# knagrecha/saturn

Measured on NVIDIA H100. Metric: candidate schedules/sec, higher is better.
Workload: dtype f32

## Files before the change

### include/saturn_b200.h

```cpp
#ifndef SATURN_B200_H
#define SATURN_B200_H

#include <stddef.h>
#include <stdint.h>

#ifdef __cplusplus
extern "C" {
#endif

#define SB_ABI_VERSION 1
#define SB_NSLOT 8
#define SB_MAX_STRATEGIES 32
#define SB_MAX_NODES 8

typedef enum sb_status {
  SB_OK = 0,
  SB_ERR_ARG = -1,
  SB_ERR_CUDA = -2,
  SB_ERR_STATE = -3,
  SB_ERR_UNSUPPORTED = -4,
  SB_ERR_NOMEM = -5
} sb_status;

#define SB_FLAG_INTEGER_STARTS 1u
// ... 78 lines not shown
  double* history_wall_s;
  int64_t* history_evaluated;
  float* history_makespan;
} sb_search_control;
typedef struct sb_search_result {
  float makespan;
  uint64_t key;
  int64_t evaluated;
  int rounds;
  int stop_reason;
  double wall_s;
} sb_search_result;
int sb_search_seed_lpt(sb_handle* h);
int sb_search_run(sb_handle* h, const sb_search_params* p, const sb_search_control* c, const uint8_t* warm_opt,
                  const void* warm_prio, uint8_t* opt_out , void* prio_out ,
                  sb_search_result* result);
int sb_search_run_multi(sb_handle** handles, int n, const sb_search_params* p, const sb_search_control* c,
                        const uint8_t* warm_opt, const void* warm_prio, uint8_t* opt_out ,
                        void* prio_out , sb_search_result* result);
int sb_search_wave(sb_handle* h, unsigned flags, int64_t* chains);
int sb_search_is_fused(sb_handle* h);
int sb_search_validate(sb_handle* h, int64_t* bad_rows);
int sb_search_verify_count(sb_handle* h, uint64_t* mismatches);
int sb_search_stats(sb_handle* h, int64_t* evaluated, int64_t* rounds_done);

#ifdef __cplusplus
}
#endif
#endif
```

### saturn_b200/_lib.py

```python
import ctypes as C
import os

_HERE = os.path.dirname(os.path.abspath(__file__))
SO_PATH = os.environ.get("SATURN_B200_LIB") or os.path.join(_HERE, "libsaturn_b200.so")

FLAG_INTEGER_STARTS = 1
FLAG_REDUCED = 2
FLAG_OPT_BY_POSITION = 4
FLAG_POST_KEY = 8
FLAG_FOLD_PREV = 16
FLAG_ALT_WARPSCAN = 32
FLAG_SUM_COMPLETION = 64
FLAG_WEIGHTED = 128
FLAG_DUE = 256
FLAG_RELEASE = 512
IPC_HANDLE_BYTES = 64
HOOK_FORCE_GENERIC = 0x80000000
HOOK_NO_STREAM = 0x40000000
HOOK_NO_FUSED = 0x20000000
HOOK_NO_INCREMENTAL = 0x10000000
HOOK_VERIFY_INCREMENTAL = 0x08000000
HOOK_ROUND1_MOVES = 0x04000000
HOOK_PLAIN_ADDR = 0x02000000
HOOK_WINDOW_BIAS = 0x01000000
HOOK_TABLE_GLOBAL = 0x00800000
HOOK_TABLE_PAIR = 0x00400000
HOOK_REORDER = 0x00200000
HOOK_NO_REORDER = 0x00100000

SYMBOLS = [
    "sb_abi_version", "sb_last_error", "sb_create", "sb_destroy", "sb_sync", "sb_set_table",
    "sb_set_sentinel", "sb_set_weights", "sb_set_due", "sb_set_release", "sb_get_reduced", "sb_eval", "sb_last_eval_path", "sb_validate", "sb_eval_host", "sb_eval_full",
    "sb_decode", "sb_xchg_create", "sb_xchg_connect", "sb_xchg_connect_local", "sb_xchg_post", "sb_xchg_reduce", "sb_xchg_check",
    "sb_search_init", "sb_search_round", "sb_search_best_key_ptr", "sb_search_best",
    "sb_search_inject", "sb_search_resample", "sb_search_seed_lpt", "sb_search_run", "sb_search_run_multi", "sb_search_wave", "sb_search_is_fused", "sb_search_stats", "sb_search_validate", "sb_search_verify_count",
]


class SearchParams(C.Structure):
    _fields_ = [("seed", C.c_uint64), ("chains", C.c_int64), ("chain_base", C.c_uint64),
                ("flags", C.c_uint), ("t_start", C.c_float), ("t_end", C.c_float),
                ("total_rounds", C.c_int), ("resample_every", C.c_int)]


class SearchControl(C.Structure):
    _fields_ = [("rounds", C.c_int), ("resample_every", C.c_int), ("sync_every", C.c_int), ("patience", C.c_int),
                ("heuristic_seeds", C.c_int), ("target_makespan", C.c_float), ("time_budget_s", C.c_double),
                ("history_cap", C.c_int), ("history_len", C.POINTER(C.c_int)),
                ("history_wall_s", C.POINTER(C.c_double)), ("history_evaluated", C.POINTER(C.c_int64)),
                ("history_makespan", C.POINTER(C.c_float))]


class SearchResultC(C.Structure):
    _fields_ = [("makespan", C.c_float), ("key", C.c_uint64), ("evaluated", C.c_int64), ("rounds", C.c_int),
                ("stop_reason", C.c_int), ("wall_s", C.c_double)]


class SaturnB200Error(RuntimeError):
# ... 33 lines not shown
        "sb_decode": [vp, vp, vp, u32, vp, vp, vp, vp, vp, vp],
        "sb_xchg_create": [vp, ci, ci, vp],
        "sb_xchg_connect": [vp, vp],
        "sb_xchg_connect_local": [C.POINTER(vp), ci],
        "sb_xchg_post": [vp, vp],
        "sb_xchg_reduce": [vp, vp, vp],
        "sb_xchg_check": [vp],
        "sb_search_init": [vp, C.POINTER(SearchParams), vp, vp],
        "sb_search_round": [vp, ci],
        "sb_search_best_key_ptr": [vp, C.POINTER(vp)],
        "sb_search_best": [vp, vp, vp, C.POINTER(C.c_float), C.POINTER(C.c_uint64)],
        "sb_search_inject": [vp, vp, vp, i64, ci],
        "sb_search_resample": [vp],
        "sb_search_seed_lpt": [vp],
        "sb_search_run": [vp, C.POINTER(SearchParams), C.POINTER(SearchControl), vp, vp, vp, vp,
                          C.POINTER(SearchResultC)],
        "sb_search_run_multi": [C.POINTER(vp), ci, C.POINTER(SearchParams), C.POINTER(SearchControl), vp, vp, vp, vp,
                                C.POINTER(SearchResultC)],
        "sb_search_wave": [vp, C.c_uint, C.POINTER(i64)],
        "sb_search_is_fused": [vp],
        "sb_search_stats": [vp, C.POINTER(i64), C.POINTER(i64)],
        "sb_search_validate": [vp, C.POINTER(i64)],
        "sb_search_verify_count": [vp, C.POINTER(C.c_uint64)],
    }
    for name, args in sigs.items():
        fn = getattr(lib, name)
        fn.argtypes = args
        fn.restype = ci
    _lib = lib
    return lib


def check(rc):
    if rc != 0:
        msg = load().sb_last_error()
        raise SaturnB200Error("saturn_b200 error %d: %s" % (rc, msg.decode() if msg else "?"))
```

### saturn_b200/csrc/sb_api.cu

```cuda
#include <math.h>
#include <stdarg.h>
#include <stdio.h>
#include <string.h>

#include <algorithm>
#include <chrono>
#include <new>
#include <string>
#include <thread>
#include <utility>
#include <vector>

#include "sb_search.h"

using namespace sb;

static thread_local char g_err[512] = "";

static int fail(int code, const char* fmt, ...) {
  va_list ap;
  va_start(ap, fmt);
  vsnprintf(g_err, sizeof(g_err), fmt, ap);
  va_end(ap);
  return code;
// ... 26 lines not shown
  bool win = false, inc = false, verify = false;
  SearchDev alloc;
  const float* w = nullptr;
  const float* due = nullptr;
  const float* rel = nullptr;
};

struct sb_handle {
  Device dev;
  cudaStream_t stream = nullptr;
  bool own_stream = false;
  int J = 0, S = 0;
  int tab_J = 0, tab_S = 0;
  int nodes = 1;
  float sentinel = kSentinel;
  float* tab = nullptr;
  float* tmin = nullptr;
  uint8_t* args = nullptr;
  uint8_t* vopt[2] = {nullptr, nullptr};
  int* nvalid[2] = {nullptr, nullptr};
  std::vector<float> h_tmin;
  std::vector<uint8_t> h_args;
  unsigned long long* d_scratch = nullptr;
  uint8_t* by_pos = nullptr;
  size_t by_pos_bytes = 0;
  cudaStream_t hs[2] = {nullptr, nullptr};
  uint8_t* st_o[2] = {nullptr, nullptr};
  uint8_t* st_p[2] = {nullptr, nullptr};
  float* st_mk[2] = {nullptr, nullptr};
  long long st_cap = 0;
  size_t st_row_o = 0, st_row_p = 0;
  uint8_t* dec_buf = nullptr;
  size_t dec_cap = 0;
  float* stage_T = nullptr;
  size_t stage_T_bytes = 0;
  float* d_w = nullptr;
  size_t d_w_cap = 0;
  std::vector<float> h_w;
  double w_sum = 0.0;
  bool has_w = false;
  float* d_d = nullptr;
  float* d_one = nullptr;
  size_t d_d_cap = 0;
  std::vector<float> h_d;
  bool has_d = false;
  float* d_r = nullptr;
// ... 87 lines not shown
  h->dev.ordinal = device;
  h->dev.sm_count = prop.multiProcessorCount;
  h->dev.smem_optin = prop.sharedMemPerBlockOptin;
  h->stream = static_cast<cudaStream_t>(stream);
  e = cudaMalloc(&h->d_scratch, 4 * sizeof(unsigned long long));
  if (e != cudaSuccess) { sb_destroy(h); return fail(SB_ERR_CUDA, "cudaMalloc: %s", cudaGetErrorString(e)); }
  for (int i = 0; i < 2; ++i) {
    e = cudaStreamCreateWithFlags(&h->hs[i], cudaStreamNonBlocking);
    if (e != cudaSuccess) { sb_destroy(h); return fail(SB_ERR_CUDA, "cudaStreamCreate: %s", cudaGetErrorString(e)); }
  }
  *out = h;
  return SB_OK;
}

int sb_destroy(sb_handle* h) {
  if (!h) return SB_OK;
  cudaSetDevice(h->dev.ordinal);
  cudaStreamSynchronize(h->stream);
  free_search(h);
  free_table(h);
  free_staging(h);
  free_xchg(h);
  cudaFree(h->d_scratch);
  cudaFree(h->by_pos);
  cudaFree(h->dec_buf);
  cudaFree(h->stage_T);
  cudaFree(h->d_w);
  cudaFree(h->d_d);
  cudaFree(h->d_one);
  cudaFree(h->d_r);
  cudaFree(h->d_rc);
  for (int i = 0; i < 2; ++i)
    if (h->hs[i]) cudaStreamDestroy(h->hs[i]);
  if (h->own_stream && h->stream) cudaStreamDestroy(h->stream);
  delete h;
  return SB_OK;
}

int sb_sync(sb_handle* h) {
  int rc = use_device(h);
  if (rc) return rc;
  CK(cudaStreamSynchronize(h->stream));
  return SB_OK;
}

int sb_set_table(sb_handle* h, const float* T, const uint8_t* gcount, int J, int S, int G, int nodes) {
// ... 287 lines not shown
      cp.opt = h->by_pos;
      int path = 5;
      CK(eval_pos_launch(h->dev, cp, h->stream, &path));
      h->last_path = 9;
      return SB_OK;
    }
  }
  if (flags & SB_FLAG_ALT_WARPSCAN) {
    if (flags & (SB_FLAG_SUM_COMPLETION | SB_FLAG_WEIGHTED | SB_FLAG_DUE | SB_FLAG_RELEASE))
      return fail(SB_ERR_UNSUPPORTED, "SB_FLAG_ALT_WARPSCAN scores the makespan without release dates only: it "
                  "cannot be combined with SB_FLAG_SUM_COMPLETION, SB_FLAG_WEIGHTED, SB_FLAG_DUE or SB_FLAG_RELEASE");
    if (flags & (SB_FLAG_POST_KEY | SB_FLAG_FOLD_PREV))
      return fail(SB_ERR_UNSUPPORTED, "SB_FLAG_ALT_WARPSCAN cannot be combined with the fused key exchange");
    cudaError_t e = eval_alt_launch(h->dev, c, h->stream);
    if (e == cudaErrorNotSupported) {
      cudaGetLastError();
      return fail(SB_ERR_UNSUPPORTED, "SB_FLAG_ALT_WARPSCAN needs one node and a table that fits in shared memory");
    }
    CK(e);
    h->last_path = 6;
    return SB_OK;
  }
  c.force_generic = (flags & HOOK_FORCE_GENERIC) ? 1 : 0;
  const bool post = (flags & SB_FLAG_POST_KEY) != 0;
  if (post) {
    if (!h->xchg_ready) return fail(SB_ERR_STATE, "SB_FLAG_POST_KEY needs sb_xchg_connect first");
    if (!best_key) return fail(SB_ERR_ARG, "SB_FLAG_POST_KEY needs best_key");
    c.xp.x = h->xd;
    c.xp.seq = ++h->xseq;
    c.xp.counter = h->d_xcounter;
    c.xp.fold_prev = (flags & SB_FLAG_FOLD_PREV) ? 1 : 0;
    c.xp.error = h->d_xerr;
  }
  CK(eval_launch(h->dev, c, h->stream, &h->last_path));
  if (post && (h->last_path == 0 || B == 0)) {
    if (c.xp.fold_prev && h->xseq > 1)
      CK(xchg_reduce_launch(h->xd, h->xseq - 1, h->d_scratch + 1, reinterpret_cast<unsigned long long*>(best_key),
                            h->d_xerr, h->stream));
    CK(xchg_post_launch(h->xd, reinterpret_cast<unsigned long long*>(best_key), h->xseq, h->stream));
  }
  return SB_OK;
}

int sb_last_eval_path(sb_handle* h) { return h ? h->last_path : -1; }

int sb_validate(sb_handle* h, const uint8_t* opt, const void* prio, int64_t B, int64_t row_stride, unsigned flags,
// ... 887 lines not shown
  CK(validate_launch(h->dev, c, h->d_scratch, h->stream, s.d.pos != 0));
  unsigned long long bad = 0;
  CK(cudaMemcpyAsync(&bad, h->d_scratch, sizeof(bad), cudaMemcpyDeviceToHost, h->stream));
  CK(cudaStreamSynchronize(h->stream));
  *bad_rows = static_cast<int64_t>(bad);
  return SB_OK;
}

int sb_search_verify_count(sb_handle* h, uint64_t* mismatches) {
  int rc = use_device(h);
  if (rc) return rc;
  if (!mismatches) return fail(SB_ERR_ARG, "mismatches is null");
  SearchState& s = h->search;
  if (!s.ready) return fail(SB_ERR_STATE, "sb_search_init has not been called");
  *mismatches = 0;
  if (!s.verify_bad) return SB_OK;
  unsigned long long v = 0;
  CK(cudaMemcpyAsync(&v, s.verify_bad, sizeof(v), cudaMemcpyDeviceToHost, h->stream));
  CK(cudaStreamSynchronize(h->stream));
  *mismatches = v;
  return SB_OK;
}

int sb_search_is_fused(sb_handle* h) { return (h && h->search.ready && h->search.fused_ok) ? 1 : 0; }

int sb_search_stats(sb_handle* h, int64_t* evaluated, int64_t* rounds_done) {
  if (!h) return fail(SB_ERR_ARG, "null handle");
  if (evaluated) *evaluated = h->search.evaluated;
  if (rounds_done) *rounds_done = h->search.rounds_done;
  return SB_OK;
}

}
```

### saturn_b200/csrc/sb_common.cuh

```cuda
#pragma once
#include <cuda_runtime.h>
#include <stdint.h>

#include "../../include/saturn_b200.h"

#if defined(__CUDA_ARCH__) && (__CUDA_ARCH__ != 900)
#error "saturn_b200 kernels target sm_90a (H100) only"
#endif

namespace sb {

constexpr int kSlots = SB_NSLOT;
constexpr int kWarp = 32;
constexpr int kMaxNodes = SB_MAX_NODES;
constexpr float kSentinel = 1.0e6f;

__device__ __forceinline__ float inf_f() { return __int_as_float(0x7f800000); }

__device__ __forceinline__ uint32_t smem_u32(const void* p) {
  return static_cast<uint32_t>(__cvta_generic_to_shared(p));
}
__device__ __forceinline__ uint32_t cluster_ctarank() {
  uint32_t r;
  asm volatile("mov.u32 %0, %%cluster_ctarank;" : "=r"(r));
// ... 26 lines not shown
  uint32_t ok;
  asm volatile(
      "{\n\t.reg .pred p;\n\t"
      "mbarrier.try_wait.parity.shared::cta.b64 p, [%1], %2;\n\t"
      "selp.u32 %0, 1, 0, p;\n\t}"
      : "=r"(ok)
      : "r"(smem_u32(bar)), "r"(parity)
      : "memory");
  return ok != 0;
}
__device__ __forceinline__ void mbar_wait(uint64_t* bar, uint32_t parity) {
  uint32_t spins = 0;
  while (!mbar_try_wait(bar, parity)) {
    if (++spins > (1u << 26)) __trap();
  }
}
__device__ __forceinline__ void tma_bulk_g2s(void* dst_smem, const void* src_gmem, uint32_t bytes,
                                             uint64_t* bar) {
  asm volatile(
      "cp.async.bulk.shared::cluster.global.mbarrier::complete_tx::bytes [%0], [%1], %2, [%3];" ::"r"(
          smem_u32(dst_smem)),
      "l"(src_gmem), "r"(bytes), "r"(smem_u32(bar))
      : "memory");
}

__device__ __forceinline__ void pmov_fma(float& dst, float src, int bit, int one) {
  int d = __float_as_int(dst);
  asm("{\n\t.reg .pred p;\n\tsetp.ne.s32 p, %2, 0;\n\t@p mad.lo.s32 %0, %1, %3, 0;\n\t}"
      : "+r"(d)
      : "r"(__float_as_int(src)), "r"(bit), "r"(one));
  dst = __int_as_float(d);
}
__device__ __forceinline__ void pinf_fma(float& dst, int bit) {
  asm("{\n\t.reg .pred p;\n\tsetp.ne.s32 p, %1, 0;\n\t@p add.f32 %0, %0, 0f7F800000;\n\t}" : "+f"(dst) : "r"(bit));
}
__device__ __forceinline__ float psel(float a, float b, int bit) {
  float r;
  asm("{\n\t.reg .pred p;\n\tsetp.ne.s32 p, %3, 0;\n\tselp.f32 %0, %1, %2, p;\n\t}" : "=f"(r) : "f"(a), "f"(b), "r"(bit));
  return r;
}

__device__ __forceinline__ float fmax3_mk(float mk, float b, float c) {
  return __int_as_float(__vimax3_s32(__float_as_int(mk), __float_as_int(b), __float_as_int(c)));
}

template <bool kIntegerStarts, bool kTrackMk = kIntegerStarts, bool kSum = false, bool kWeighted = false,
// ... 58 lines not shown
```

### saturn_b200/csrc/sb_eval.cu

```cuda
#include "sb_lane.cuh"

namespace sb {

struct TileArgs {
  const float* tab;
  int J, SG;
  const uint8_t* opt;
  const uint8_t* prio;
  long long B;
  long long stride_o, stride_p;
  int row_o, row_p;
  int copy_o, copy_p;
  int use_bulk;
  int nodes;
  float* out;
  unsigned long long* best_key;
  uint32_t id_base;
  long long ntiles;
  int one;
  SearchFuse sf;
  XchgPost xp;
  const float* w;
  const float* d;
  const float* r;
};

template <int PB, bool INT, bool STREAM, bool MULTI, bool SEARCH = false, bool TABG = false, int ADDR = 0,
          bool SUM = false, bool W = false, bool D = false, bool R = false>
__global__ void __launch_bounds__(STREAM ? 512 : 384, 1) k_eval_tiles(const TileArgs a) {
  static_assert(!(SEARCH && (STREAM || TABG)), "the fused search round runs on shared-memory tiles only");
  static_assert(ADDR == 0 || (!TABG && !MULTI && !SEARCH), "ADDR = 1 needs the table and the opt rows in shared memory");
  static_assert(SUM || !W, "weights scale the sum of completion times only");
  static_assert(W || !D, "due dates run on the weighted form");
  extern __shared__ __align__(128) uint8_t smem[];
  const int nw = blockDim.x >> 5;
  const int warp = threadIdx.x >> 5, lane = threadIdx.x & 31;
  const uint32_t tab_bytes = TABG ? 0u : static_cast<uint32_t>(a.J) * a.SG * 4u;
  const uint32_t w_bytes = (W && !TABG) ? ((static_cast<uint32_t>(a.J) * 4u + 15u) & ~15u) : 0u;
  const uint32_t d_bytes = D ? w_bytes : 0u;
  const uint32_t r_bytes = (R && !TABG) ? ((static_cast<uint32_t>(a.J) * 4u + 15u) & ~15u) : 0u;
  float* tab_s = reinterpret_cast<float*>(smem);
  [[maybe_unused]] float* w_s = reinterpret_cast<float*>(smem + tab_bytes);
  [[maybe_unused]] float* d_s = reinterpret_cast<float*>(smem + tab_bytes + w_bytes);
  [[maybe_unused]] float* r_s = reinterpret_cast<float*>(smem + tab_bytes + w_bytes + d_bytes);
  uint64_t* bars = reinterpret_cast<uint64_t*>(smem + ((tab_bytes + w_bytes + d_bytes + r_bytes + 15u) & ~15u));
  uint8_t* tiles = reinterpret_cast<uint8_t*>(bars) + (((1 + nw) * 8 + 15) & ~15);
  const uint32_t node_bytes = MULTI ? static_cast<uint32_t>(a.nodes) * 1024u : 0u;
// ... 88 lines not shown
    unsigned long long k = ~0ull;
    bool ok = true;
    if (lane < a.xp.x.world) {
      const unsigned long long* slot = a.xp.x.peer[lane] + (want & 1ull) * 2;
      unsigned long long seen;
      unsigned spins = 0;
      for (;;) {
        asm volatile("ld.acquire.sys.global.u64 %0, [%1];" : "=l"(seen) : "l"(slot + 1) : "memory");
        if (seen >= want || !block || ++spins >= (1u << 22)) break;
        __nanosleep(64);
      }
      ok = seen >= want;
      if (ok) asm volatile("ld.relaxed.sys.global.u64 %0, [%1];" : "=l"(k) : "l"(slot) : "memory");
    }
    ok = __all_sync(0xffffffffu, ok);
    if (!ok) {
      if (block && lane == 0) *a.xp.error = 1;
      return;
    }
    fold_keys(k);
  };
  if (fold_pending) look_issue();

  uint32_t phase = 0;
  bool tab_ready = TABG;
  for (long long tile = static_cast<long long>(blockIdx.x) * nw + warp; tile < a.ntiles;
       tile += static_cast<long long>(gridDim.x) * nw) {
    const long long b0 = tile * 32;
    if (!SEARCH && fold_pending) {
      look_consume();
      if (fold_pending) look_issue();
    }
    const long long cand = (SEARCH && a.sf.deal) ? lane * a.ntiles + tile : b0 + lane;
    const bool active = cand < a.B;
    const int nb = SEARCH ? __popc(__ballot_sync(0xffffffffu, active)) : static_cast<int>(min(32ll, a.B - b0));
    const uint8_t* pg = a.prio + cand * a.stride_p;
    __syncwarp();
    PrioChunk q;
    if (a.use_bulk) {
      fence_proxy_async();
      if (lane == 0)
        mbar_arrive_expect_tx(bar_w, static_cast<uint32_t>(nb) * (a.copy_o + (STREAM ? 0 : a.copy_p)));
      __syncwarp();
      if (active) {
        tma_bulk_g2s(tile_o + lane * a.row_o, a.opt + cand * a.stride_o, a.copy_o, bar_w);
        if (!STREAM) tma_bulk_g2s(tile_p + lane * a.row_p, pg, a.copy_p, bar_w);
      }
      if (STREAM && active) q = ld_prio32<true>(pg);
      mbar_wait(bar_w, phase);
      phase ^= 1;
    } else {
      for (int r = 0; r < nb; ++r) {
        const uint8_t* so = a.opt + (b0 + r) * a.stride_o;
        const uint8_t* sp = a.prio + (b0 + r) * a.stride_p;
        for (int x = lane; x < a.J; x += 32) tile_o[r * a.row_o + x] = so[x];
        for (int x = lane; x < a.J * PB; x += 32) tile_p[r * a.row_p + x] = sp[x];
      }
      __syncwarp();
    }
    if (!tab_ready) {
      mbar_wait(bar_tab, 0);
      tab_ready = true;
    }
    auto evaluate = [&](const uint8_t* prio_row_s) -> float {
      st.reset(a.nodes);
      const int J = a.J;
      if constexpr (STREAM && ADDR == 1) {
        constexpr int STEPS = 32;
        constexpr int kBatch = 8;
        const int nch = (J + STEPS - 1) / STEPS, nfull = J / STEPS;
        uint32_t ob[kBatch];
        float rb[kBatch];
        [[maybe_unused]] float wb[kBatch];
// ... 1 lines not shown
        [[maybe_unused]] float xb[kBatch];
        auto resolve = [&](const uint32_t* w) {
          int js[kBatch];
#pragma unroll
          for (int i = 0; i < kBatch; ++i) js[i] = prio_at<1>(w, i);
#pragma unroll
          for (int i = 0; i < kBatch; ++i) ob[i] = st.gather_opt(js[i]);
#pragma unroll
          for (int i = 0; i < kBatch; ++i) rb[i] = st.gather_rt(js[i], ob[i]);
          if constexpr (W) {
#pragma unroll
            for (int i = 0; i < kBatch; ++i) wb[i] = st.gather_w(js[i]);
          }
          if constexpr (D) {
#pragma unroll
            for (int i = 0; i < kBatch; ++i) db[i] = st.gather_d(js[i]);
          }
          if constexpr (R) {
#pragma unroll
            for (int i = 0; i < kBatch; ++i) xb[i] = st.gather_r(js[i]);
          }
        };
        if (nfull > 0) resolve(q.w);
        for (int c = 0; c < nfull; ++c) {
          PrioChunk nxt = q;
          if (c + 1 < nch) nxt = ld_prio32<true>(pg + (c + 1) * 32);
          const bool ahead = c + 1 < nfull;
          uint32_t head[kBatch / 4];
#pragma unroll
          for (int i = 0; i < kBatch / 4; ++i) head[i] = ahead ? nxt.w[i] : q.w[i];
#pragma unroll
          for (int b = 0; b < STEPS / kBatch; ++b) {
            uint32_t oc[kBatch];
            float rc[kBatch];
            [[maybe_unused]] float wc[kBatch];
            [[maybe_unused]] float dc[kBatch];
            [[maybe_unused]] float xc[kBatch];
#pragma unroll
            for (int i = 0; i < kBatch; ++i) { oc[i] = ob[i]; rc[i] = rb[i]; }
            if constexpr (W) {
#pragma unroll
              for (int i = 0; i < kBatch; ++i) wc[i] = wb[i];
            }
            if constexpr (D) {
#pragma unroll
              for (int i = 0; i < kBatch; ++i) dc[i] = db[i];
            }
            if constexpr (R) {
#pragma unroll
              for (int i = 0; i < kBatch; ++i) xc[i] = xb[i];
            }
            resolve(b + 1 < STEPS / kBatch ? q.w + (b + 1) * (kBatch / 4) : head);
#pragma unroll
            for (int i = 0; i < kBatch; ++i) {
              const float x = R ? xc[i] : 0.f;
              if constexpr (D) st.step_resolved(static_cast<int>(oc[i]), rc[i], i & 1, wc[i], dc[i], x);
              else if constexpr (W) st.step_resolved(static_cast<int>(oc[i]), rc[i], i & 1, wc[i], 0.f, x);
              else st.step_resolved(static_cast<int>(oc[i]), rc[i], i & 1, 0.f, 0.f, x);
            }
          }
          q = nxt;
        }
        if (nfull < nch) {
          const int rem = J - nfull * STEPS;
#pragma unroll
          for (int t = 0; t < STEPS; ++t)
            if (t < rem) st.step(prio_at<1>(q.w, t), t & 1);
        }
      } else if (STREAM) {
        constexpr int STEPS = 32 / PB;
        const int nch = (J + STEPS - 1) / STEPS;
        for (int c = 0; c < nch; ++c) {
          PrioChunk nxt = q;
          if (c + 1 < nch) nxt = ld_prio32<true>(pg + (c + 1) * 32);
          if ((c + 1) * STEPS <= J) {
#pragma unroll
            for (int t = 0; t < STEPS; ++t) st.step(prio_at<PB>(q.w, t), t & 1);
          } else {
            const int rem = J - c * STEPS;
#pragma unroll
            for (int t = 0; t < STEPS; ++t)
              if (t < rem) st.step(prio_at<PB>(q.w, t), t & 1);
          }
          q = nxt;
        }
      } else {
        const uint4* prow = reinterpret_cast<const uint4*>(prio_row_s);
        constexpr int STEPS = 16 / PB;
        const int nch = (J + STEPS - 1) / STEPS;
        for (int c = 0; c < nch; ++c) {
          const uint4 p = prow[c];
          const uint32_t w[4] = {p.x, p.y, p.z, p.w};
          if ((c + 1) * STEPS <= J) {
#pragma unroll
            for (int t = 0; t < STEPS; ++t) st.step(prio_at<PB>(w, t), t & 1);
          } else {
            const int rem = J - c * STEPS;
#pragma unroll
            for (int t = 0; t < STEPS; ++t)
              if (t < rem) st.step(prio_at<PB>(w, t), t & 1);
          }
        }
      }
      return st.result();
    };
    [[maybe_unused]] auto eval_from = [&](const uint8_t* prio_row_s, int w0, uint32_t par, bool save,
                                          float* snap_t) -> float {
// ... 20 lines not shown
          for (int i = 0; i < 8; ++i) __stcg(sp + i * 32, st.f[i]);
          __stcg(sp + 8 * 32, st.running());
        }
        const uint4 p = prow[c];
        const uint32_t wd[4] = {p.x, p.y, p.z, p.w};
        if ((c + 1) * STEPS <= J) {
#pragma unroll
          for (int t = 0; t < STEPS; ++t) st.step(prio_at<PB>(wd, t), t & 1);
        } else {
          const int rem = J - c * STEPS;
#pragma unroll 1
          for (int t = 0; t < rem; ++t) st.step(PB == 1 ? prio_row_s[c * STEPS + t] : reinterpret_cast<const uint16_t*>(prio_row_s)[c * STEPS + t], -1);
        }
      }
      return st.result();
    };
    if (!SEARCH) {
      float mk = 0.f;
      if (active) {
        mk = evaluate(tile_p + lane * a.row_p);
        a.out[b0 + lane] = mk;
      }
      if (a.best_key != nullptr) fold_best(a.best_key, active, mk, a.id_base + static_cast<uint32_t>(b0 + lane), lane);
    } else {
      const long long c = cand;
      const int rl = active ? lane : 0;
      uint8_t* orow_s = tile_o + rl * a.row_o;
      uint8_t* prow_s = tile_p + rl * a.row_p;
      st.orow = orow_s;
      const uint64_t gid = a.sf.chain_base + static_cast<uint64_t>(c);
      float cm = active ? a.sf.cur_mk[c] : 0.f;
      bool moving = active;
      const bool inc = !MULTI && a.sf.snap != nullptr;
      const bool win = !MULTI && a.sf.win != 0;
      const int nwin = (a.J + kSnapPos - 1) / kSnapPos;
      float* snap_t = inc ? a.sf.snap + static_cast<size_t>(tile) * (static_cast<size_t>(nwin - 1) * 2 * 9 * 32) : nullptr;
      uint32_t par = 0;
      const uint32_t inc_bits = launch_incumbent_bits(a.sf);
#pragma unroll 1
      for (int r = inc ? -1 : 0; r < a.sf.nrounds; ++r) {
        const int round = a.sf.round + r;
        const bool fill = r < 0;
        if (!fill && a.sf.resample_every > 0 && round > 1 && (round - 1) % a.sf.resample_every == 0) {
          const uint64_t rr = rng_u64(a.sf.seed ^ 0x7e57a11ull, gid, static_cast<uint64_t>(round));
          const int rival = static_cast<int>(rr >> 59);
          const float rcm = __shfl_sync(0xffffffffu, cm, rival);
// ... 80 lines not shown
            const uint64_t rr = rng_u64(a.sf.seed, gid, 4ull * round + 3);
            const float u = (static_cast<uint32_t>(rr >> 40) + 0.5f) * (1.0f / 16777216.0f);
            acc = u < __expf(-(mk - cm) / temp);
          }
          if (acc) {
            if (mv.kind != 0) {
              write_back<PB>(mv, orow_s, prow_s, a.sf.cur_o + c * a.stride_o, a.sf.cur_p + c * a.stride_p);
              a.sf.cur_mk[c] = mk;
              cm = mk;
              if (inc) par ^= (w0 + 1 < nwin) ? (~0u << w0) : 0u;
            }
          } else {
            undo_move<PB>(mv, orow_s, prow_s);
            mk = cm;
          }
        }
        if (a.best_key != nullptr) fold_best(a.best_key, active, mk, a.id_base + static_cast<uint32_t>(c), lane);
        if (active && __float_as_uint(mk) < inc_bits) moving = false;
      }
      st.orow = tile_o + lane * a.row_o;
    }
  }
  if (!tab_ready && threadIdx.x == 0) mbar_wait(bar_tab, 0);
  if (!SEARCH && fold_pending) try_fold(true);
  if (SEARCH) {
    if (a.sf.keep.counter != nullptr) keep_best_tail(a.sf);
    return;
  }
  if (a.xp.counter != nullptr) {
    __syncthreads();
    if (threadIdx.x == 0) {
      __threadfence();
      const unsigned done = atomicAdd(a.xp.counter, 1u);
      if (done == gridDim.x - 1) {
        *a.xp.counter = 0;
        __threadfence();
        const unsigned long long k = *reinterpret_cast<volatile unsigned long long*>(a.best_key);
        unsigned long long* slot = a.xp.x.local + (a.xp.seq & 1ull) * 2;
        asm volatile("st.relaxed.sys.global.u64 [%0], %1;" ::"l"(slot), "l"(k) : "memory");
        asm volatile("st.release.sys.global.u64 [%0], %1;" ::"l"(slot + 1), "l"(a.xp.seq) : "memory");
      }
    }
  }
}

struct GenericArgs {
// ... 215 lines not shown
  tp->smem = tab_bytes + (((1 + nw) * 8 + 15) & ~15) + nw * per_warp;
  return nw;
}

using TileKernel = void (*)(TileArgs);

static bool bulk_aligned(const EvalCall& c) {
  return (c.stride_o % 16 == 0) && (c.stride_p % 16 == 0) && (reinterpret_cast<uintptr_t>(c.opt) % 16 == 0) &&
         (reinterpret_cast<uintptr_t>(c.prio) % 16 == 0);
}

static TileArgs tile_args(const EvalCall& c, const TilePlan& tp) {
  TileArgs a;
  a.tab = c.tab; a.J = c.J; a.SG = c.SG; a.opt = c.opt; a.prio = c.prio; a.B = c.B;
  a.stride_o = c.stride_o; a.stride_p = c.stride_p;
  a.row_o = tp.row_o; a.row_p = tp.row_p; a.copy_o = tp.copy_o; a.copy_p = tp.copy_p;
  a.nodes = c.nodes;
  a.out = c.out; a.best_key = c.best_key; a.id_base = c.id_base;
  a.w = c.w;
  a.d = c.d;
  a.r = c.r;
  a.ntiles = (c.B + 31) / 32;
  a.one = 1;
  return a;
}

static cudaError_t launch_tiles(const Device& dev, TileKernel kern, const TileArgs& a, const TilePlan& tp,
                                cudaStream_t st) {
  long long ctas = (a.ntiles + tp.warps - 1) / tp.warps;
  int grid = static_cast<int>(ctas < dev.sm_count ? ctas : dev.sm_count);
  return launch(kern, grid, tp.warps * 32, tp.smem, st, a);
}

cudaError_t eval_launch(const Device& dev, const EvalCall& c, cudaStream_t st, int* path_used) {
  if (c.B <= 0) return cudaSuccess;
  const int pb = c.J <= 256 ? 1 : 2;
  const bool multi = c.nodes > 1;
  const bool bulk_ok = bulk_aligned(c);
  const bool stream_ok = bulk_ok && (c.stride_p % 32 == 0) && (reinterpret_cast<uintptr_t>(c.prio) % 32 == 0) &&
                         !(c.flags & HOOK_NO_STREAM);
  const int arrays = job_arrays(c.flags);
  TilePlan tp;
  int nw = 0;
  bool stream = false, tabg = false;
  if (!c.force_generic) {
    if (stream_ok) {
      nw = plan_tiles(dev, c.J, c.SG, pb, true, c.nodes, &tp, false, arrays);
      stream = nw >= 2 && c.stride_o >= tp.copy_o && c.stride_p >= ((c.J * pb + 31) & ~31);
      if (!stream && !multi) {
        nw = plan_tiles(dev, c.J, c.SG, pb, true, c.nodes, &tp, true);
        stream = tabg = nw >= 2 && c.stride_o >= tp.copy_o && c.stride_p >= ((c.J * pb + 31) & ~31);
      }
    }
    if (!stream) nw = plan_tiles(dev, c.J, c.SG, pb, false, c.nodes, &tp, false, arrays);
  }
  if (nw >= 2) {
    TileArgs a = tile_args(c, tp);
    a.use_bulk = stream || (bulk_ok && (c.stride_o >= tp.copy_o) && (c.stride_p >= tp.copy_p));
    a.xp = c.xp;
    if (path_used) *path_used = tabg ? 4 : (stream ? 3 : (a.use_bulk ? 2 : 1));
    const bool fma_addr = pb == 1 && stream && !tabg && !multi && !(c.flags & HOOK_PLAIN_ADDR);
    const TileKernel kern = with_eval_types(pb, c.flags, [&](auto PB, auto INT, auto SUM, auto W, auto D, auto R) -> TileKernel {
      if (tabg) return k_eval_tiles<PB, INT, true, false, false, true, 0, SUM, W, D, R>;
      if constexpr (PB == 1) {
        if (fma_addr) return k_eval_tiles<1, INT, true, false, false, false, 1, SUM, W, D, R>;
      }
      return with_bool(stream, [&](auto STREAM) {
        return with_bool(multi, [&](auto MULTI) -> TileKernel {
          return k_eval_tiles<PB, INT, STREAM, MULTI, false, false, 0, SUM, W, D, R>;
        });
      });
    });
    return launch_tiles(dev, kern, a, tp, st);
  }
  GenericArgs g;
  g.tab = c.tab; g.J = c.J; g.SG = c.SG; g.opt = c.opt; g.prio = c.prio; g.B = c.B;
  g.stride_o = c.stride_o; g.stride_p = c.stride_p; g.out = c.out; g.best_key = c.best_key;
  g.id_base = c.id_base; g.tab_in_smem = 0; g.nodes = c.nodes; g.one = 1; g.w = c.w; g.d = c.d; g.r = c.r;
  if (path_used) *path_used = 0;
  const size_t tab_bytes = static_cast<size_t>(c.J) * c.SG * 4;
  size_t smem = multi ? static_cast<size_t>(4) * c.nodes * 1024u : 0u;
  if (tab_bytes <= dev.smem_optin / 2) {
    g.tab_in_smem = 1;
    smem += tab_bytes;
// ... 68 lines not shown
```

### saturn_b200/csrc/sb_internal.h

```cpp
#pragma once
#include <cuda_runtime.h>
#include <stdint.h>

#include <type_traits>

#include "sb_common.cuh"

namespace sb {

enum : unsigned {
  HOOK_FORCE_GENERIC = 0x80000000u,
  HOOK_NO_STREAM = 0x40000000u,
  HOOK_NO_FUSED = 0x20000000u,
  HOOK_NO_INCREMENTAL = 0x10000000u,
  HOOK_VERIFY_INCREMENTAL = 0x08000000u,
  HOOK_ROUND1_MOVES = 0x04000000u,
  HOOK_PLAIN_ADDR = 0x02000000u,
  HOOK_WINDOW_BIAS = 0x01000000u,
  HOOK_TABLE_GLOBAL = 0x00800000u,
  HOOK_TABLE_PAIR = 0x00400000u,
  HOOK_REORDER = 0x00200000u,
  HOOK_NO_REORDER = 0x00100000u,
};
static_assert(((HOOK_FORCE_GENERIC | HOOK_NO_STREAM | HOOK_NO_FUSED | HOOK_NO_INCREMENTAL | HOOK_VERIFY_INCREMENTAL |
                HOOK_ROUND1_MOVES | HOOK_PLAIN_ADDR | HOOK_WINDOW_BIAS | HOOK_TABLE_GLOBAL | HOOK_TABLE_PAIR |
                HOOK_REORDER | HOOK_NO_REORDER) &
               (SB_FLAG_INTEGER_STARTS | SB_FLAG_REDUCED | SB_FLAG_OPT_BY_POSITION | SB_FLAG_POST_KEY |
                SB_FLAG_FOLD_PREV | SB_FLAG_ALT_WARPSCAN | SB_FLAG_SUM_COMPLETION | SB_FLAG_WEIGHTED |
                SB_FLAG_DUE | SB_FLAG_RELEASE)) == 0,
              "the test hooks share no bit with the SB_FLAG_* flags");

template <class F>
decltype(auto) with_bool(bool b, F&& f) {
  return b ? f(std::true_type{}) : f(std::false_type{});
}
template <class F>
decltype(auto) with_pb(int pb, F&& f) {
  return pb == 1 ? f(std::integral_constant<int, 1>{}) : f(std::integral_constant<int, 2>{});
}
template <class F>
decltype(auto) with_eval_types(int pb, unsigned flags, F&& f) {
  return with_pb(pb, [&](auto PB) {
    return with_bool(flags & SB_FLAG_INTEGER_STARTS, [&](auto INT) {
      return with_bool(flags & SB_FLAG_RELEASE, [&](auto R) {
        return with_bool(flags & SB_FLAG_SUM_COMPLETION, [&](auto SUM) {
          if constexpr (SUM) {
            return with_bool(flags & (SB_FLAG_WEIGHTED | SB_FLAG_DUE), [&](auto W) {
              if constexpr (W) return with_bool(flags & SB_FLAG_DUE, [&](auto D) { return f(PB, INT, SUM, W, D, R); });
              else return f(PB, INT, SUM, W, std::false_type{}, R);
            });
          } else {
            return f(PB, INT, SUM, std::false_type{}, std::false_type{}, R);
          }
// ... 45 lines not shown
struct TilePlan {
  int warps = 0;
  int row_o = 0, row_p = 0, copy_o = 0, copy_p = 0;
  size_t smem = 0;
};

struct EvalCall {
  const float* tab = nullptr;
  const float* w = nullptr;
  const float* d = nullptr;
  const float* r = nullptr;
  int J = 0, SG = 0;
  const uint8_t* opt = nullptr;
  const uint8_t* prio = nullptr;
  long long B = 0;
  long long stride_o = 0, stride_p = 0;
  unsigned flags = 0;
  int nodes = 1;
  float* out = nullptr;
  unsigned long long* best_key = nullptr;
  uint32_t id_base = 0;
  int force_generic = 0;
  XchgPost xp;
};

constexpr int kMaxFusedRounds = 16;
constexpr int kSnapPos = 32;
struct SearchFuse {
  float* cur_mk = nullptr;
  uint8_t* cur_o = nullptr;
  uint8_t* cur_p = nullptr;
  const uint8_t* vopt = nullptr;
  const int* nvalid = nullptr;
  uint64_t seed = 0, chain_base = 0;
  int round = 0;
  int nrounds = 1;
  int nodes = 1;
  float temperature[kMaxFusedRounds] = {};
  int resample_every = 0;
  int deal = 0;
  int win = 0;
  int win_bias = 0;
  float* snap = nullptr;
  unsigned long long* verify_bad = nullptr;
  struct KeepBest {
    unsigned* counter = nullptr;
// ... 23 lines not shown
```

### saturn_b200/engine.py

```python
from __future__ import annotations

import ctypes as C
from typing import Optional, Sequence, Tuple

import numpy as np
import torch

from . import _lib
from ._lib import FLAG_INTEGER_STARTS, FLAG_REDUCED, SaturnB200Error, SearchParams, check

NSLOT = 8


OBJECTIVES = ("makespan", "completion", "weighted_completion", "tardiness", "weighted_tardiness")


def objective_flag(objective: str) -> int:
    if objective not in OBJECTIVES:
        from .solver import SolverError
        raise SolverError("objective must be one of %s, not %r" % (", ".join(map(repr, OBJECTIVES)), objective))
    if objective == "makespan":
        return 0
    return _lib.FLAG_SUM_COMPLETION | (_lib.FLAG_WEIGHTED if objective.startswith("weighted_") else 0) | (
        _lib.FLAG_DUE if objective.endswith("tardiness") else 0)
# ... 175 lines not shown
    def _check_cands(self, opt: torch.Tensor, prio: torch.Tensor, on_device: bool):
        if opt.dtype != torch.uint8:
            raise TypeError("opt must be uint8")
        if prio.dtype != self.prio_dtype:
            raise TypeError("prio must be %s for J=%d" % (self.prio_dtype, self.J))
        if opt.dim() != 2 or prio.dim() != 2 or opt.shape != prio.shape:
            raise ValueError("opt / prio must both be [B][J]")
        if opt.shape[1] != self.J:
            raise ValueError("candidates have %d jobs, table has %d" % (opt.shape[1], self.J))
        if opt.stride(1) != 1 or prio.stride(1) != 1 or (opt.shape[0] > 1 and opt.stride(0) != prio.stride(0)):
            raise ValueError("opt / prio rows must be contiguous with the same row stride")
        if on_device and (opt.device != self.device or prio.device != self.device):
            raise ValueError("candidates must live on %s" % self.device)
        if not on_device and (opt.is_cuda or prio.is_cuda):
            raise ValueError("host evaluation takes CPU tensors")
        B = opt.shape[0]
        stride = opt.stride(0) if B > 1 else max(opt.stride(0), self.J)
        return B, stride

    def eval(self, opt: torch.Tensor, prio: torch.Tensor, integer_starts: bool = True, reduced: bool = False,
             out: Optional[torch.Tensor] = None, best_key: Optional[torch.Tensor] = None, id_base: int = 0,
             _force_generic: bool = False, _no_stream: bool = False, post_key: bool = False, fold_prev: bool = False,
             by_position: bool = False, _plain_addr: bool = False, alt_shape: bool = False,
             _table_home: int = 0, _reorder: Optional[bool] = None, objective: str = "makespan") -> torch.Tensor:
        B, stride = self._check_cands(opt, prio, True)
        if out is None:
            out = torch.empty(B, dtype=torch.float32, device=self.device)
        fl = self._flags(integer_starts, reduced, objective) | (_lib.HOOK_FORCE_GENERIC if _force_generic else 0) | (
            _lib.HOOK_NO_STREAM if _no_stream else 0) | (_lib.HOOK_PLAIN_ADDR if _plain_addr else 0) | (
            _lib.FLAG_POST_KEY if post_key else 0) | (
            _lib.FLAG_FOLD_PREV if (post_key and fold_prev) else 0) | (
            _lib.FLAG_OPT_BY_POSITION if by_position else 0) | (_lib.FLAG_ALT_WARPSCAN if alt_shape else 0) | (
            {0: 0, 1: _lib.HOOK_TABLE_GLOBAL, 2: _lib.HOOK_TABLE_PAIR}[_table_home]) | (
            0 if _reorder is None else (_lib.HOOK_REORDER if _reorder else _lib.HOOK_NO_REORDER))
        kp = C.c_void_p(best_key.data_ptr()) if best_key is not None else None
        check(self._lib.sb_eval(self._h, C.c_void_p(opt.data_ptr()), C.c_void_p(prio.data_ptr()), B, stride, fl,
                                C.c_void_p(out.data_ptr()), kp, id_base & 0xffffffff))
        return out

    def last_eval_path(self) -> int:
        return int(self._lib.sb_last_eval_path(self._h))

    def validate(self, opt: torch.Tensor, prio: torch.Tensor, reduced: bool = False) -> int:
        B, stride = self._check_cands(opt, prio, True)
        bad = C.c_int64(0)
        check(self._lib.sb_validate(self._h, C.c_void_p(opt.data_ptr()), C.c_void_p(prio.data_ptr()), B, stride,
                                    _flags(False, reduced), C.byref(bad)))
        return int(bad.value)

    def eval_host(self, opt: torch.Tensor, prio: torch.Tensor, integer_starts: bool = True, reduced: bool = False,
                  out: Optional[torch.Tensor] = None, objective: str = "makespan") -> torch.Tensor:
        B, stride = self._check_cands(opt, prio, False)
        if out is None:
            out = torch.empty(B, dtype=torch.float32, pin_memory=True)
        check(self._lib.sb_eval_host(self._h, C.c_void_p(opt.data_ptr()), C.c_void_p(prio.data_ptr()), B, stride,
                                     self._flags(integer_starts, reduced, objective), C.c_void_p(out.data_ptr())))
        return out

    def eval_full(self, opt: torch.Tensor, prio: torch.Tensor, integer_starts: bool = True, reduced: bool = False,
                  objective: str = "makespan"):
        B, stride = self._check_cands(opt, prio, True)
# ... 330 lines not shown
```

Before: 1.937 billion.

## Use single packed bulk copy per tile and stagger warps with named barriers

When candidate rows are densely packed, lane 0 issues one bulk TMA copy for the whole tile instead of one copy per lane. Warps are also phase-staggered with named barriers on the first tile so their prio loads and compute don't all contend at once. The aim is to cut per-row copy overhead and smooth memory bursts. Debug hooks add optional globaltimer-based wait measurement and switches to disable either feature. The barrier gating adds sync overhead and deadlock risk if the counts are wrong.

```diff
diff --git a/include/saturn_b200.h b/include/saturn_b200.h
--- a/include/saturn_b200.h
+++ b/include/saturn_b200.h
@@ -124,6 +124,8 @@
 int sb_search_is_fused(sb_handle* h);
 int sb_search_validate(sb_handle* h, int64_t* bad_rows);
 int sb_search_verify_count(sb_handle* h, uint64_t* mismatches);
+int sb_debug_tile_options(sb_handle* h, unsigned options);
+int sb_debug_tile_wait(sb_handle* h, uint64_t* out);
 int sb_search_stats(sb_handle* h, int64_t* evaluated, int64_t* rounds_done);
 
 #ifdef __cplusplus
diff --git a/saturn_b200/_lib.py b/saturn_b200/_lib.py
--- a/saturn_b200/_lib.py
+++ b/saturn_b200/_lib.py
@@ -27,6 +27,9 @@
 HOOK_TABLE_PAIR = 0x00400000
 HOOK_REORDER = 0x00200000
 HOOK_NO_REORDER = 0x00100000
+TILE_DEBUG_TIMING = 1
+TILE_DEBUG_ROW_COPIES = 2
+TILE_DEBUG_NO_STAGGER = 4
 
 SYMBOLS = [
     "sb_abi_version", "sb_last_error", "sb_create", "sb_destroy", "sb_sync", "sb_set_table",
@@ -34,6 +37,7 @@
     "sb_decode", "sb_xchg_create", "sb_xchg_connect", "sb_xchg_connect_local", "sb_xchg_post", "sb_xchg_reduce", "sb_xchg_check",
     "sb_search_init", "sb_search_round", "sb_search_best_key_ptr", "sb_search_best",
     "sb_search_inject", "sb_search_resample", "sb_search_seed_lpt", "sb_search_run", "sb_search_run_multi", "sb_search_wave", "sb_search_is_fused", "sb_search_stats", "sb_search_validate", "sb_search_verify_count",
+    "sb_debug_tile_options", "sb_debug_tile_wait",
 ]
 
 
@@ -113,6 +117,8 @@
         "sb_search_stats": [vp, C.POINTER(i64), C.POINTER(i64)],
         "sb_search_validate": [vp, C.POINTER(i64)],
         "sb_search_verify_count": [vp, C.POINTER(C.c_uint64)],
+        "sb_debug_tile_options": [vp, C.c_uint],
+        "sb_debug_tile_wait": [vp, C.POINTER(C.c_uint64)],
     }
     for name, args in sigs.items():
         fn = getattr(lib, name)
diff --git a/saturn_b200/csrc/sb_api.cu b/saturn_b200/csrc/sb_api.cu
--- a/saturn_b200/csrc/sb_api.cu
+++ b/saturn_b200/csrc/sb_api.cu
@@ -72,6 +72,8 @@
   std::vector<float> h_tmin;
   std::vector<uint8_t> h_args;
   unsigned long long* d_scratch = nullptr;
+  unsigned tile_debug = 0;
+  unsigned long long* d_tile_wait = nullptr;
   uint8_t* by_pos = nullptr;
   size_t by_pos_bytes = 0;
   cudaStream_t hs[2] = {nullptr, nullptr};
@@ -205,6 +207,7 @@
   free_staging(h);
   free_xchg(h);
   cudaFree(h->d_scratch);
+  cudaFree(h->d_tile_wait);
   cudaFree(h->by_pos);
   cudaFree(h->dec_buf);
   cudaFree(h->stage_T);
@@ -538,6 +541,14 @@
     return SB_OK;
   }
   c.force_generic = (flags & HOOK_FORCE_GENERIC) ? 1 : 0;
+  c.tile_debug = h->tile_debug;
+  if (h->tile_debug & TILE_DEBUG_TIMING) {
+    if (!h->d_tile_wait) {
+      CK(cudaMalloc(&h->d_tile_wait, 2 * sizeof(unsigned long long)));
+      CK(cudaMemsetAsync(h->d_tile_wait, 0, 2 * sizeof(unsigned long long), h->stream));
+    }
+    c.tile_wait = h->d_tile_wait;
+  }
   const bool post = (flags & SB_FLAG_POST_KEY) != 0;
   if (post) {
     if (!h->xchg_ready) return fail(SB_ERR_STATE, "SB_FLAG_POST_KEY needs sb_xchg_connect first");
@@ -1471,6 +1482,29 @@
   return SB_OK;
 }
 
+int sb_debug_tile_options(sb_handle* h, unsigned options) {
+  if (!h) return fail(SB_ERR_ARG, "null handle");
+  if (options & ~(TILE_DEBUG_TIMING | TILE_DEBUG_ROW_COPIES | TILE_DEBUG_NO_STAGGER))
+    return fail(SB_ERR_ARG, "unknown tile debug option 0x%x", options);
+  h->tile_debug = options;
+  return SB_OK;
+}
+
+int sb_debug_tile_wait(sb_handle* h, uint64_t* out) {
+  int rc = use_device(h);
+  if (rc) return rc;
+  if (!out) return fail(SB_ERR_ARG, "out is null");
+  unsigned long long v[2] = {0ull, 0ull};
+  if (h->d_tile_wait) {
+    CK(cudaMemcpyAsync(v, h->d_tile_wait, sizeof(v), cudaMemcpyDeviceToHost, h->stream));
+    CK(cudaMemsetAsync(h->d_tile_wait, 0, sizeof(v), h->stream));
+    CK(cudaStreamSynchronize(h->stream));
+  }
+  out[0] = v[0];
+  out[1] = v[1];
+  return SB_OK;
+}
+
 int sb_search_is_fused(sb_handle* h) { return (h && h->search.ready && h->search.fused_ok) ? 1 : 0; }
 
 int sb_search_stats(sb_handle* h, int64_t* evaluated, int64_t* rounds_done) {
diff --git a/saturn_b200/csrc/sb_common.cuh b/saturn_b200/csrc/sb_common.cuh
--- a/saturn_b200/csrc/sb_common.cuh
+++ b/saturn_b200/csrc/sb_common.cuh
@@ -72,6 +72,17 @@
           smem_u32(dst_smem)),
       "l"(src_gmem), "r"(bytes), "r"(smem_u32(bar))
       : "memory");
+}
+__device__ __forceinline__ void named_arrive(uint32_t id, uint32_t count) {
+  asm volatile("barrier.cta.arrive %0, %1;" ::"r"(id), "r"(count) : "memory");
+}
+__device__ __forceinline__ void named_sync(uint32_t id, uint32_t count) {
+  asm volatile("barrier.cta.sync %0, %1;" ::"r"(id), "r"(count) : "memory");
+}
+__device__ __forceinline__ unsigned long long globaltimer_ns() {
+  unsigned long long t;
+  asm volatile("mov.u64 %0, %%globaltimer;" : "=l"(t));
+  return t;
 }
 
 __device__ __forceinline__ void pmov_fma(float& dst, float src, int bit, int one) {
diff --git a/saturn_b200/csrc/sb_eval.cu b/saturn_b200/csrc/sb_eval.cu
--- a/saturn_b200/csrc/sb_eval.cu
+++ b/saturn_b200/csrc/sb_eval.cu
@@ -23,6 +23,9 @@
   const float* w;
   const float* d;
   const float* r;
+  int packed;
+  int stagger;
+  unsigned long long* tile_wait;
 };
 
 template <int PB, bool INT, bool STREAM, bool MULTI, bool SEARCH = false, bool TABG = false, int ADDR = 0,
@@ -157,10 +160,27 @@
   };
   if (fold_pending) look_issue();
 
+  constexpr bool kFetch = STREAM && !MULTI && !TABG && !SEARCH;
+  const long long tstride = static_cast<long long>(gridDim.x) * nw;
+  const int nfull_ch = a.J / (32 / PB);
+  int nph = 1;
+  if (kFetch && a.stagger && static_cast<long long>(blockIdx.x) * nw + tstride + nw - 1 < a.ntiles)
+    nph = min(min(4, nw), (nfull_ch + 1) / 2);
+  auto gate_count = [&](int p) { return 32u * (1u + static_cast<uint32_t>((nw - 1 - p) / nph + 1)); };
+  int arrive_at = nfull_ch + 1;
+  if (nph > 1) {
+    if (warp == 0) {
+      arrive_at = 1;
+    } else if (warp % nph != 0) {
+      named_sync(warp % nph, gate_count(warp % nph));
+    }
+  }
+  unsigned long long t_wait = 0ull, t_loop = 0ull;
+  if (kFetch && a.tile_wait != nullptr) t_loop = globaltimer_ns();
+
   uint32_t phase = 0;
   bool tab_ready = TABG;
-  for (long long tile = static_cast<long long>(blockIdx.x) * nw + warp; tile < a.ntiles;
-       tile += static_cast<long long>(gridDim.x) * nw) {
+  for (long long tile = static_cast<long long>(blockIdx.x) * nw + warp; tile < a.ntiles; tile += tstride) {
     const long long b0 = tile * 32;
     if (!SEARCH && fold_pending) {
       look_consume();
@@ -173,17 +193,22 @@
     __syncwarp();
     PrioChunk q;
     if (a.use_bulk) {
+      unsigned long long t_fetch = 0ull;
+      if (kFetch && a.tile_wait != nullptr) t_fetch = globaltimer_ns();
       fence_proxy_async();
       if (lane == 0)
         mbar_arrive_expect_tx(bar_w, static_cast<uint32_t>(nb) * (a.copy_o + (STREAM ? 0 : a.copy_p)));
       __syncwarp();
-      if (active) {
+      if (kFetch && a.packed) {
+        if (lane == 0) tma_bulk_g2s(tile_o, a.opt + b0 * a.stride_o, static_cast<uint32_t>(nb) * a.copy_o, bar_w);
+      } else if (active) {
         tma_bulk_g2s(tile_o + lane * a.row_o, a.opt + cand * a.stride_o, a.copy_o, bar_w);
         if (!STREAM) tma_bulk_g2s(tile_p + lane * a.row_p, pg, a.copy_p, bar_w);
       }
       if (STREAM && active) q = ld_prio32<true>(pg);
       mbar_wait(bar_w, phase);
       phase ^= 1;
+      if (kFetch && a.tile_wait != nullptr) t_wait += globaltimer_ns() - t_fetch;
     } else {
       for (int r = 0; r < nb; ++r) {
         const uint8_t* so = a.opt + (b0 + r) * a.stride_o;
@@ -231,7 +256,9 @@
           }
         };
         if (nfull > 0) resolve(q.w);
-        for (int c = 0; c < nfull; ++c) {
+        int c = 0, stop = min(arrive_at, nfull);
+        for (;;) {
+        for (; c < stop; ++c) {
           PrioChunk nxt = q;
           if (c + 1 < nch) nxt = ld_prio32<true>(pg + (c + 1) * 32);
           const bool ahead = c + 1 < nfull;
@@ -270,6 +297,10 @@
           }
           q = nxt;
         }
+        if (stop >= nfull) break;
+        named_arrive(stop, gate_count(stop));
+        stop = stop + 1 < nph ? stop + 1 : nfull;
+        }
         if (nfull < nch) {
           const int rem = J - nfull * STEPS;
 #pragma unroll
@@ -279,7 +310,9 @@
       } else if (STREAM) {
         constexpr int STEPS = 32 / PB;
         const int nch = (J + STEPS - 1) / STEPS;
-        for (int c = 0; c < nch; ++c) {
+        int c = 0, stop = min(arrive_at, nch);
+        for (;;) {
+        for (; c < stop; ++c) {
           PrioChunk nxt = q;
           if (c + 1 < nch) nxt = ld_prio32<true>(pg + (c + 1) * 32);
           if ((c + 1) * STEPS <= J) {
@@ -292,6 +325,10 @@
               if (t < rem) st.step(prio_at<PB>(q.w, t), t & 1);
           }
           q = nxt;
+        }
+        if (stop >= nch) break;
+        named_arrive(stop, gate_count(stop));
+        stop = stop + 1 < nph ? stop + 1 : nch;
         }
       } else {
         const uint4* prow = reinterpret_cast<const uint4*>(prio_row_s);
@@ -358,6 +395,7 @@
         a.out[b0 + lane] = mk;
       }
       if (a.best_key != nullptr) fold_best(a.best_key, active, mk, a.id_base + static_cast<uint32_t>(b0 + lane), lane);
+      arrive_at = nfull_ch + 1;
     } else {
       const long long c = cand;
       const int rl = active ? lane : 0;
@@ -484,6 +522,10 @@
     }
   }
   if (!tab_ready && threadIdx.x == 0) mbar_wait(bar_tab, 0);
+  if (kFetch && a.tile_wait != nullptr && lane == 0) {
+    atomicAdd(a.tile_wait, t_wait);
+    atomicAdd(a.tile_wait + 1, globaltimer_ns() - t_loop);
+  }
   if (!SEARCH && fold_pending) try_fold(true);
   if (SEARCH) {
     if (a.sf.keep.counter != nullptr) keep_best_tail(a.sf);
@@ -745,6 +787,8 @@
   a.r = c.r;
   a.ntiles = (c.B + 31) / 32;
   a.one = 1;
+  a.packed = a.stagger = 0;
+  a.tile_wait = nullptr;
   return a;
 }
 
@@ -783,6 +827,12 @@
     a.xp = c.xp;
     if (path_used) *path_used = tabg ? 4 : (stream ? 3 : (a.use_bulk ? 2 : 1));
     const bool fma_addr = pb == 1 && stream && !tabg && !multi && !(c.flags & HOOK_PLAIN_ADDR);
+    if (stream && !tabg && !multi) {
+      a.packed = c.stride_o == tp.copy_o && c.stride_p == tp.copy_p && !(c.tile_debug & TILE_DEBUG_ROW_COPIES);
+      if (a.packed) a.row_o = tp.copy_o;
+      a.stagger = !(c.tile_debug & TILE_DEBUG_NO_STAGGER);
+      a.tile_wait = c.tile_wait;
+    }
     const TileKernel kern = with_eval_types(pb, c.flags, [&](auto PB, auto INT, auto SUM, auto W, auto D, auto R) -> TileKernel {
       if (tabg) return k_eval_tiles<PB, INT, true, false, false, true, 0, SUM, W, D, R>;
       if constexpr (PB == 1) {
diff --git a/saturn_b200/csrc/sb_internal.h b/saturn_b200/csrc/sb_internal.h
--- a/saturn_b200/csrc/sb_internal.h
+++ b/saturn_b200/csrc/sb_internal.h
@@ -29,6 +29,12 @@
                 SB_FLAG_FOLD_PREV | SB_FLAG_ALT_WARPSCAN | SB_FLAG_SUM_COMPLETION | SB_FLAG_WEIGHTED |
                 SB_FLAG_DUE | SB_FLAG_RELEASE)) == 0,
               "the test hooks share no bit with the SB_FLAG_* flags");
+
+enum TileDebug : unsigned {
+  TILE_DEBUG_TIMING = 1u,
+  TILE_DEBUG_ROW_COPIES = 2u,
+  TILE_DEBUG_NO_STAGGER = 4u,
+};
 
 template <class F>
 decltype(auto) with_bool(bool b, F&& f) {
@@ -120,6 +126,8 @@
   uint32_t id_base = 0;
   int force_generic = 0;
   XchgPost xp;
+  unsigned tile_debug = 0;
+  unsigned long long* tile_wait = nullptr;
 };
 
 constexpr int kMaxFusedRounds = 16;
diff --git a/saturn_b200/engine.py b/saturn_b200/engine.py
--- a/saturn_b200/engine.py
+++ b/saturn_b200/engine.py
@@ -221,7 +221,8 @@
              out: Optional[torch.Tensor] = None, best_key: Optional[torch.Tensor] = None, id_base: int = 0,
              _force_generic: bool = False, _no_stream: bool = False, post_key: bool = False, fold_prev: bool = False,
              by_position: bool = False, _plain_addr: bool = False, alt_shape: bool = False,
-             _table_home: int = 0, _reorder: Optional[bool] = None, objective: str = "makespan") -> torch.Tensor:
+             _table_home: int = 0, _reorder: Optional[bool] = None, objective: str = "makespan",
+             _tile_debug: int = 0) -> torch.Tensor:
         B, stride = self._check_cands(opt, prio, True)
         if out is None:
             out = torch.empty(B, dtype=torch.float32, device=self.device)
@@ -233,9 +234,20 @@
             {0: 0, 1: _lib.HOOK_TABLE_GLOBAL, 2: _lib.HOOK_TABLE_PAIR}[_table_home]) | (
             0 if _reorder is None else (_lib.HOOK_REORDER if _reorder else _lib.HOOK_NO_REORDER))
         kp = C.c_void_p(best_key.data_ptr()) if best_key is not None else None
-        check(self._lib.sb_eval(self._h, C.c_void_p(opt.data_ptr()), C.c_void_p(prio.data_ptr()), B, stride, fl,
-                                C.c_void_p(out.data_ptr()), kp, id_base & 0xffffffff))
+        if _tile_debug:
+            check(self._lib.sb_debug_tile_options(self._h, int(_tile_debug)))
+        try:
+            check(self._lib.sb_eval(self._h, C.c_void_p(opt.data_ptr()), C.c_void_p(prio.data_ptr()), B, stride, fl,
+                                    C.c_void_p(out.data_ptr()), kp, id_base & 0xffffffff))
+        finally:
+            if _tile_debug:
+                check(self._lib.sb_debug_tile_options(self._h, 0))
         return out
+
+    def debug_tile_wait(self):
+        v = (C.c_uint64 * 2)()
+        check(self._lib.sb_debug_tile_wait(self._h, v))
+        return int(v[0]), int(v[1])
 
     def last_eval_path(self) -> int:
         return int(self._lib.sb_last_eval_path(self._h))
```

After: 2.071 billion (median of 6 runs). +6.9%, better.
